# cliangyu/video-diffusion

Measured on AMD Instinct MI355X. Metric: denoise-steps/sec, higher is better.
Workload: dtype f32

## Files before the change

### video-diffusion_amd/csrc/attn_temporal.hip

```cpp
#include "vd_common.h"
#include <cstdlib>
#include <string>

namespace vd {

__device__ __forceinline__ float dot4(f32x4 a, f32x4 b) { return a.x * b.x + a.y * b.y + a.z * b.z + a.w * b.w; }

template <int PB, int TMAX, bool RPE>
__global__ __launch_bounds__(256) void attn_temporal_kernel(AttnTemporalArgs a) {
    extern __shared__ __attribute__((aligned(16))) float smem[];
    const int T = a.T, C = a.C, HW = a.HW, C3 = 3 * a.C;
    const int F = C / a.heads, F4 = F >> 2, FP = F + 4, TS = T + 1;
    float* qs = smem;
    float* ks = qs + PB * T * FP;
    float* sc = ks + PB * T * FP;
    const int b = blockIdx.z, h = blockIdx.y, p0 = blockIdx.x * PB;
    const int np = min(PB, HW - p0);
    const int tid = threadIdx.x;
    const float* qkv_b = a.qkv + (size_t)b * T * HW * C3 + h * F;

    for (int idx = tid; idx < PB * T * F4; idx += 256) {
        const int f4 = idx % F4, r = idx / F4;
        const int t = r % T, p = r / T;
        const float* src = qkv_b + ((size_t)t * HW + p0 + min(p, np - 1)) * C3 + f4 * 4;
        f32x4 q = *reinterpret_cast<const f32x4*>(src) * a.scale;
        f32x4 k = *reinterpret_cast<const f32x4*>(src + C);
        if (p >= np) { q = f32x4{0.f, 0.f, 0.f, 0.f}; k = q; }
        *reinterpret_cast<f32x4*>(qs + (p * T + t) * FP + f4 * 4) = q;
        *reinterpret_cast<f32x4*>(ks + (p * T + t) * FP + f4 * 4) = k;
    }
    __syncthreads();

    for (int pr = tid; pr < T * T; pr += 256) {
        const int t = pr / T, s = pr - t * T;
        float acc[PB];
#pragma unroll
        for (int p = 0; p < PB; ++p) acc[p] = 0.f;
        const float* rk = RPE ? a.Rk + (((size_t)b * T + t) * T + s) * C + h * F : nullptr;
        const float* rq = RPE ? a.Rq + (((size_t)b * T + s) * T + t) * C + h * F : nullptr;
        const float* qrow = qs + t * FP;
        const float* krow = ks + s * FP;
#pragma unroll 3
        for (int f0 = 0; f0 < F; f0 += 8) {
            f32x4 rk0, rk1, rq0, rq1;
            if constexpr (RPE) {
                rk0 = *reinterpret_cast<const f32x4*>(rk + f0); rk1 = *reinterpret_cast<const f32x4*>(rk + f0 + 4);
                rq0 = *reinterpret_cast<const f32x4*>(rq + f0) * a.scale; rq1 = *reinterpret_cast<const f32x4*>(rq + f0 + 4) * a.scale;
            }
#pragma unroll
            for (int p = 0; p < PB; ++p) {
                const f32x4 q0 = *reinterpret_cast<const f32x4*>(qrow + p * T * FP + f0);
                const f32x4 q1 = *reinterpret_cast<const f32x4*>(qrow + p * T * FP + f0 + 4);
                const f32x4 k0 = *reinterpret_cast<const f32x4*>(krow + p * T * FP + f0);
                const f32x4 k1 = *reinterpret_cast<const f32x4*>(krow + p * T * FP + f0 + 4);
                if constexpr (RPE)
                    acc[p] += dot4(q0, k0 + rk0) + dot4(q1, k1 + rk1) + dot4(k0, rq0) + dot4(k1, rq1);
                else
                    acc[p] += dot4(q0, k0) + dot4(q1, k1);
            }
        }
        bool masked = false;
        if (a.mask) {
            const float mt = a.mask[b * T + t], ms = a.mask[b * T + s];
            float allowed = mt * ms;
            if (a.allow_pad) allowed += (1.f - mt) * (1.f - ms);
            else if (t == s) allowed = 1.f;
            masked = allowed == 0.f;
        }
#pragma unroll
        for (int p = 0; p < PB; ++p) sc[(p * T + t) * TS + s] = masked ? -INFINITY : acc[p];
    }
    __syncthreads();

    for (int row = tid; row < np * T; row += 256) {
        float* r = sc + row * TS;
        float mx = -INFINITY;
        for (int s = 0; s < T; ++s) mx = fmaxf(mx, r[s]);
        float sum = 0.f;
        for (int s = 0; s < T; ++s) { const float e = __expf(r[s] - mx); r[s] = e; sum += e; }
        const float inv = 1.0f / sum;
        for (int s = 0; s < T; ++s) r[s] *= inv;
    }
    __syncthreads();

    for (int item = tid; item < T * F4; item += 256) {
        const int t = item / F4, f4 = item - t * F4;
        f32x4 rv[TMAX];
#pragma unroll
        for (int s = 0; s < TMAX; ++s) {
            rv[s] = f32x4{0.f, 0.f, 0.f, 0.f};
            if constexpr (RPE)
                rv[s] = *reinterpret_cast<const f32x4*>(a.Rv + (((size_t)b * T + t) * T + min(s, T - 1)) * C + h * F + f4 * 4);
        }
        for (int p = 0; p < np; ++p) {
            const float* ar = sc + (p * T + t) * TS;
            const float* vbase = qkv_b + 2 * C + (size_t)(p0 + p) * C3 + f4 * 4;
            f32x4 o = {0.f, 0.f, 0.f, 0.f};
#pragma unroll
            for (int s = 0; s < TMAX; ++s) {
                const f32x4 v = *reinterpret_cast<const f32x4*>(vbase + (size_t)min(s, T - 1) * HW * C3);
                const float w = s < T ? ar[min(s, T - 1)] : 0.f;
                o += (v + rv[s]) * w;
            }
            *reinterpret_cast<f32x4*>(a.out + (((size_t)b * T + t) * HW + p0 + p) * C + h * F + f4 * 4) = o;
        }
    }
}

#ifdef VD_ATT_TIMING
__device__ unsigned long long g_att_stamp[16];
#define ATT_STAMP(i)                                                                                   \
    do {                                                                                               \
        if (threadIdx.x == 0 && blockIdx.x == 3 && blockIdx.y == 1 && blockIdx.z == 2) {               \
            __builtin_amdgcn_sched_barrier(0);                                                         \
            g_att_stamp[i] = __builtin_amdgcn_s_memrealtime();                                         \
            __builtin_amdgcn_sched_barrier(0);                                                         \
        }                                                                                              \
    } while (0)
extern "C" int vd_debug_att_stamps(unsigned long long* host_out) {
    return (int)hipMemcpyFromSymbol(host_out, HIP_SYMBOL(g_att_stamp), sizeof(g_att_stamp));
}
#else
#define ATT_STAMP(i)
#endif

__device__ __forceinline__ f32x4 mfma4(float x, float y, f32x4 c) { return __builtin_amdgcn_mfma_f32_16x16x4f32(x, y, c, 0, 0, 0); }

__device__ __forceinline__ void rows_regs_transpose(float& x0, float& x1, float& x2, float& x3) {
    auto u = [](float f) { return __builtin_bit_cast(unsigned, f); };
    auto f = [](unsigned v) { return __builtin_bit_cast(float, v); };
    auto p01 = __builtin_amdgcn_permlane16_swap(u(x0), u(x1), false, false);
    auto p23 = __builtin_amdgcn_permlane16_swap(u(x2), u(x3), false, false);
    auto q02 = __builtin_amdgcn_permlane32_swap(p01[0], p23[0], false, false);
    auto q13 = __builtin_amdgcn_permlane32_swap(p01[1], p23[1], false, false);
    x0 = f(q02[0]); x2 = f(q02[1]); x1 = f(q13[0]); x3 = f(q13[1]);
}

template <int NT, int JM, bool RPE, bool EXACT>
__global__ __launch_bounds__(512, 2) void attn_temporal_mfma_kernel(AttnTemporalArgs a) {
    constexpr int TP = 16 * NT, RS = TP + 1, PS = TP * RS + (NT == 1 ? 1 : 17);
    extern __shared__ __attribute__((aligned(16))) float smem[];
    float* w = smem;
    const int T = EXACT ? 16 * NT : a.T, C = a.C, HW = a.HW, C3 = 3 * a.C;
    const int F = C / a.heads, NJ = EXACT ? JM : F >> 4;
    const int b = blockIdx.z, h = blockIdx.y, p0 = blockIdx.x * 16;
    const int tid = threadIdx.x, wv = tid >> 6, l = tid & 63, i16 = l & 15, g = l >> 4;
    const float* qb = a.qkv + ((size_t)b * T * HW + p0) * C3 + h * F;
    auto row = [&](int t, int px) { return qb + ((size_t)t * HW + px) * C3; };
    auto ld4 = [](const float* p) { return *reinterpret_cast<const f32x4*>(p); };
    const int tcl[2] = {min(i16, T - 1), min(16 + i16, T - 1)};
    const f32x4 zero4 = {0.f, 0.f, 0.f, 0.f};

    ATT_STAMP(0);
    constexpr int JG = NT == 1 ? 2 : 1, NG = JM / JG, NU = 2 * NT;
    constexpr bool AHEAD = NT == 1;
    struct Ops { f32x4 qa1[2][NT][JG], kb1[2][NT][JG], xa2[NU][JG], rb2[NU][NT][JG], xa3[NU][JG], rb3[NU][NT][JG]; };
    f32x4 acc1[2][NT][NT], acc2[NU][NT], acc3[NU][NT];
#pragma unroll
    for (int u = 0; u < 2; ++u)
#pragma unroll
        for (int m = 0; m < NT; ++m)
#pragma unroll
            for (int n = 0; n < NT; ++n) acc1[u][m][n] = zero4;
#pragma unroll
    for (int u = 0; u < NU; ++u)
#pragma unroll
        for (int n = 0; n < NT; ++n) { acc2[u][n] = zero4; acc3[u][n] = zero4; }
    const float* q1[2][NT];
#pragma unroll
    for (int u = 0; u < 2; ++u)
#pragma unroll
        for (int m = 0; m < NT; ++m) q1[u][m] = row(tcl[m], 2 * wv + u) + 4 * g;
    const float* rkq[NT];
#pragma unroll
    for (int n = 0; n < NT; ++n) rkq[n] = (size_t)b * T * T * C + (size_t)tcl[n] * C + h * F + 4 * g + (const float*)nullptr;
    auto request = [&](Ops& o, int grp, bool own, bool rel) {
#pragma unroll
        for (int jj = 0; jj < JG; ++jj) {
            const int j = grp * JG + jj;
            if (EXACT || j < NJ) {
                if (own) {
#pragma unroll
                    for (int u = 0; u < 2; ++u)
#pragma unroll
                        for (int m = 0; m < NT; ++m) { o.qa1[u][m][jj] = ld4(q1[u][m] + 16 * j); o.kb1[u][m][jj] = ld4(q1[u][m] + C + 16 * j); }
                }
                if constexpr (RPE) {
#pragma unroll
                    for (int u = 0; u < (rel ? NU : 0); ++u) {
                        const int t = wv + 8 * u;
                        if (EXACT || t < T) {
                            const float* xr = row(t, i16) + 4 * g + 16 * j;
                            o.xa2[u][jj] = ld4(xr);
                            o.xa3[u][jj] = ld4(xr + C);
#pragma unroll
                            for (int n = 0; n < NT; ++n) {
                                const size_t ro = (size_t)(rkq[n] - (const float*)nullptr) + (size_t)t * T * C + 16 * j;
                                o.rb2[u][n][jj] = ld4(a.Rk + ro);
                                o.rb3[u][n][jj] = ld4(a.Rq + ro);
                            }
                        }
                    }
                }
            }
        }
    };
    auto products = [&](const Ops& o, int grp, bool own, bool rel) {
#pragma unroll
        for (int jj = 0; jj < JG; ++jj) {
            if (EXACT || grp * JG + jj < NJ) {
#pragma unroll
                for (int e = 0; e < 4; ++e) {
#pragma unroll
                    for (int u = 0; u < (own ? 2 : 0); ++u)
#pragma unroll
                        for (int m = 0; m < NT; ++m)
#pragma unroll
                            for (int n = 0; n < NT; ++n) acc1[u][m][n] = mfma4(o.qa1[u][m][jj][e] * a.scale, o.kb1[u][n][jj][e], acc1[u][m][n]);
                    if constexpr (RPE) {
#pragma unroll
                        for (int u = 0; u < (rel ? NU : 0); ++u)
                            if (EXACT || wv + 8 * u < T) {
#pragma unroll
                                for (int n = 0; n < NT; ++n) {
                                    acc2[u][n] = mfma4(o.xa2[u][jj][e] * a.scale, o.rb2[u][n][jj][e], acc2[u][n]);
                                    acc3[u][n] = mfma4(o.xa3[u][jj][e], o.rb3[u][n][jj][e] * a.scale, acc3[u][n]);
                                }
                            }
                    }
                }
            }
        }
    };
    if constexpr (AHEAD) {
        Ops o[2];
        request(o[0], 0, true, true);
#pragma unroll
        for (int grp = 0; grp < NG; ++grp) {
            if (grp + 1 < NG) request(o[(grp + 1) & 1], grp + 1, true, true);
            __builtin_amdgcn_sched_barrier(0);
            products(o[grp & 1], grp, true, true);
            __builtin_amdgcn_sched_barrier(0);
        }
    } else {
#pragma unroll 1
        for (int grp = 0; grp < NG; ++grp) {
            Ops o;
            request(o, grp, true, false);
            products(o, grp, true, false);
            if constexpr (RPE) {
                request(o, grp, false, true);
                products(o, grp, false, true);
            }
        }
    }
    ATT_STAMP(1);
#pragma unroll
    for (int u = 0; u < 2; ++u)
#pragma unroll
        for (int m = 0; m < NT; ++m)
#pragma unroll
            for (int n = 0; n < NT; ++n)
#pragma unroll
                for (int r = 0; r < 4; ++r) w[(2 * wv + u) * PS + (16 * m + 4 * g + r) * RS + 16 * n + i16] = acc1[u][m][n][r];
    __syncthreads();
    if constexpr (RPE) {
#pragma unroll
        for (int u = 0; u < NU; ++u) {
            const int t = wv + 8 * u;
            if (t < T) {
#pragma unroll
                for (int n = 0; n < NT; ++n)
#pragma unroll
                    for (int r = 0; r < 4; ++r) w[(4 * g + r) * PS + t * RS + 16 * n + i16] += acc2[u][n][r];
            }
        }
        __syncthreads();
#pragma unroll
        for (int u = 0; u < NU; ++u) {
            const int sk = wv + 8 * u;
            if (sk < T) {
#pragma unroll
                for (int n = 0; n < NT; ++n)
#pragma unroll
                    for (int r = 0; r < 4; ++r) w[(4 * g + r) * PS + (16 * n + i16) * RS + sk] += acc3[u][n][r];
            }
        }
        __syncthreads();
    }

    ATT_STAMP(2);
    for (int rix = tid; rix < 16 * TP; rix += 512) {
        const int px = rix / TP, t = rix - px * TP;
        float* r = w + px * PS + t * RS;
        if (t >= T) {
            for (int s = 0; s < TP; ++s) r[s] = 0.f;
            continue;
        }
        float mx = -INFINITY;
        const float mt = a.mask ? a.mask[b * T + t] : 1.f;
        for (int s = 0; s < T; ++s) {
            float v = r[s];
            if (a.mask) {
                const float ms = a.mask[b * T + s];
                float allowed = mt * ms;
                if (a.allow_pad) allowed += (1.f - mt) * (1.f - ms);
                else if (t == s) allowed = 1.f;
                if (allowed == 0.f) v = -INFINITY;
            }
            r[s] = v;
            mx = fmaxf(mx, v);
        }
        float sum = 0.f;
        for (int s = 0; s < T; ++s) { const float e = __expf(r[s] - mx); r[s] = e; sum += e; }
        const float inv = 1.0f / sum;
        for (int s = 0; s < T; ++s) r[s] *= inv;
        for (int s = T; s < TP; ++s) r[s] = 0.f;
    }
    __syncthreads();

    ATT_STAMP(3);
    const int KS = (T + 3) >> 2;
    if (EXACT ? wv < JM : wv < NJ) {
        const int f0 = 16 * wv + i16;
        const float* vb = qb + 2 * C + f0;
        const float* rvb = RPE ? a.Rv + ((size_t)b * T) * T * C + h * F + f0 : nullptr;
#pragma unroll 1
        for (int m = 0; m < NT; ++m) {
            if (16 * m >= T) break;
            float rr[NT == 1 ? 4 : 1][16];
            f32x4 acc[16];
#pragma unroll
            for (int px = 0; px < 16; ++px) acc[px] = zero4;
#pragma unroll 1
            for (int kc = 0; kc < NT; ++kc) {
                if (16 * kc >= T) break;
                float vr[4][16];
#pragma unroll
                for (int k4 = 0; k4 < 4; ++k4)
                    if (EXACT || 4 * kc + k4 < KS) {
                        const float* vs = vb + (size_t)min(16 * kc + 4 * k4 + g, T - 1) * HW * C3;
#pragma unroll
                        for (int px = 0; px < 16; ++px) vr[k4][px] = vs[(size_t)px * C3];
                    }
                if constexpr (RPE && NT == 1) {
#pragma unroll
                    for (int k4 = 0; k4 < 4; ++k4)
                        if (EXACT || k4 < KS) {
                            const float* rv = rvb + (size_t)min(4 * k4 + g, T - 1) * C;
#pragma unroll
                            for (int tl = 0; tl < 16; ++tl) rr[k4][tl] = rv[(size_t)min(tl, T - 1) * T * C];
                        }
                }
                __builtin_amdgcn_sched_barrier(0);
#pragma unroll
                for (int k4 = 0; k4 < 4; ++k4)
                    if (EXACT || 4 * kc + k4 < KS) {
                        const float* ar = w + (16 * m + i16) * RS + 16 * kc + 4 * k4 + g;
#pragma unroll
                        for (int px = 0; px < 16; ++px) acc[px] = mfma4(ar[px * PS], vr[k4][px], acc[px]);
                    }
            }
            ATT_STAMP(4);
            f32x4 res[16];
#pragma unroll
            for (int bq = 0; bq < 4; ++bq)
#pragma unroll
                for (int d = 0; d < 4; ++d) {
                    float x0 = acc[bq][d], x1 = acc[4 + bq][d], x2 = acc[8 + bq][d], x3 = acc[12 + bq][d];
                    rows_regs_transpose(x0, x1, x2, x3);
                    res[d][bq] = x0; res[4 + d][bq] = x1; res[8 + d][bq] = x2; res[12 + d][bq] = x3;
                }
            if constexpr (RPE) {
                if constexpr (NT == 1) {
#pragma unroll
                    for (int k4 = 0; k4 < 4; ++k4)
                        if (EXACT || k4 < KS) {
                            const float* ar = w + i16 * PS + 4 * k4 + g;
#pragma unroll
                            for (int tl = 0; tl < 16; ++tl) res[tl] = mfma4(ar[tl * RS], rr[k4][tl], res[tl]);
                        }
                } else {
#pragma unroll 1
                    for (int kc = 0; kc < NT; ++kc) {
                        if (16 * kc >= T) break;
                        float r4[4][16];
#pragma unroll
                        for (int k4 = 0; k4 < 4; ++k4)
                            if (4 * kc + k4 < KS) {
                                const float* rv = rvb + (size_t)min(16 * kc + 4 * k4 + g, T - 1) * C;
#pragma unroll
                                for (int tl = 0; tl < 16; ++tl) r4[k4][tl] = rv[(size_t)min(16 * m + tl, T - 1) * T * C];
                            }
#pragma unroll
                        for (int k4 = 0; k4 < 4; ++k4)
                            if (4 * kc + k4 < KS) {
                                const float* ar = w + i16 * PS + (16 * m) * RS + 16 * kc + 4 * k4 + g;
#pragma unroll
                                for (int tl = 0; tl < 16; ++tl) res[tl] = mfma4(ar[tl * RS], r4[k4][tl], res[tl]);
                            }
                    }
                }
            }
            ATT_STAMP(5);
#pragma unroll
            for (int tl = 0; tl < 16; ++tl) {
                const int t = 16 * m + tl;
                if (t < T) {
                    float* o = a.out + (((size_t)b * T + t) * HW + p0 + 4 * g) * C + h * F + f0;
#pragma unroll
                    for (int r = 0; r < 4; ++r) o[(size_t)r * C] = res[tl][r];
                }
            }
        }
    }
    ATT_STAMP(6);
}

template <int NT, int JM, bool RPE, bool EXACT>
static int launch_tm(const AttnTemporalArgs& a, hipStream_t s) {
    constexpr int TP = 16 * NT, PS = TP * (TP + 1) + (NT == 1 ? 1 : 17);
    constexpr size_t lds = (size_t)16 * PS * sizeof(float);
    if (lds > 48 * 1024) VD_RAISE_LDS((&attn_temporal_mfma_kernel<NT, JM, RPE, EXACT>), lds);
    dim3 grid(a.HW / 16, a.heads, a.B);
    hipLaunchKernelGGL((attn_temporal_mfma_kernel<NT, JM, RPE, EXACT>), grid, dim3(512), lds, s, a);
    VD_HIP(hipGetLastError());
    return 0;
}

template <int PB, int TMAX, bool RPE>
static int launch_tt(const AttnTemporalArgs& a, size_t lds, hipStream_t s) {
    VD_RAISE_LDS((&attn_temporal_kernel<PB, TMAX, RPE>), lds);
    dim3 grid((a.HW + PB - 1) / PB, a.heads, a.B);
    hipLaunchKernelGGL((attn_temporal_kernel<PB, TMAX, RPE>), grid, dim3(256), lds, s, a);
    VD_HIP(hipGetLastError());
    return 0;
}

int launch_attn_temporal(const AttnTemporalArgs& a, hipStream_t s) {
    VD_REQUIRE(a.T >= 1 && a.T <= kMaxWindowFrames, "temporal window of 1..128 frames");
    VD_REQUIRE(a.C % a.heads == 0 && (a.C / a.heads) % 8 == 0, "head dim multiple of 8");
    VD_REQUIRE((a.Rk == nullptr) == (a.Rq == nullptr) && (a.Rk == nullptr) == (a.Rv == nullptr), "all or no RPE terms");
    if (a.T > 32) return launch_attn_temporal_long(a, s);
    const int F = a.C / a.heads;
    if (a.HW % 16 == 0 && F % 16 == 0 && F <= 128) {
        const bool rpe = a.Rk != nullptr;
        if (a.T == 16 && F == 96) return rpe ? launch_tm<1, 6, true, true>(a, s) : launch_tm<1, 6, false, true>(a, s);
        if (a.T == 16 && F == 128) return rpe ? launch_tm<1, 8, true, true>(a, s) : launch_tm<1, 8, false, true>(a, s);
        if (a.T <= 16) {
            if (F <= 64) return rpe ? launch_tm<1, 4, true, false>(a, s) : launch_tm<1, 4, false, false>(a, s);
            return rpe ? launch_tm<1, 8, true, false>(a, s) : launch_tm<1, 8, false, false>(a, s);
        }
        if (F <= 64) return rpe ? launch_tm<2, 4, true, false>(a, s) : launch_tm<2, 4, false, false>(a, s);
        return rpe ? launch_tm<2, 8, true, false>(a, s) : launch_tm<2, 8, false, false>(a, s);
    }
    auto lds_for = [&](int pb) { return ((size_t)2 * pb * a.T * (F + 4) + (size_t)pb * a.T * (a.T + 1)) * sizeof(float); };
    const bool rpe = a.Rk != nullptr;
    const bool big = lds_for(4) > 96 * 1024;
    VD_REQUIRE(lds_for(2) <= 150 * 1024, "head dim too large for the temporal attention tile");
    if (a.T <= 16) {
        if (big) return rpe ? launch_tt<2, 16, true>(a, lds_for(2), s) : launch_tt<2, 16, false>(a, lds_for(2), s);
        return rpe ? launch_tt<4, 16, true>(a, lds_for(4), s) : launch_tt<4, 16, false>(a, lds_for(4), s);
    }
    if (big) return rpe ? launch_tt<2, 32, true>(a, lds_for(2), s) : launch_tt<2, 32, false>(a, lds_for(2), s);
    return rpe ? launch_tt<4, 32, true>(a, lds_for(4), s) : launch_tt<4, 32, false>(a, lds_for(4), s);
}

}
```

Before: 49.81.

## Add low-register DUO path for exact T=16 RPE temporal attention

For the exact T=16, RPE, single-tile configuration, the kernel now targets 4 blocks per CU instead of 2. To fit that register budget it uses 32-bit byte offsets for addressing, halves the per-group operand staging, and reuses one buffer for the Rk/Rq operands. The AV and RPE-V phase is rewritten as a 16-stage software pipeline that prefetches one stage ahead and does the transpose in the middle. Dispatch now falls back to the generic path when tensor sizes exceed 32-bit offsets. Risks are register spilling and reduced load-ahead depth hurting latency hiding.

```diff
diff --git a/video-diffusion_amd/csrc/attn_temporal.hip b/video-diffusion_amd/csrc/attn_temporal.hip
--- a/video-diffusion_amd/csrc/attn_temporal.hip
+++ b/video-diffusion_amd/csrc/attn_temporal.hip
@@ -1,6 +1,7 @@
 #include "vd_common.h"
 #include <cstdlib>
 #include <string>
+#include <type_traits>
 
 namespace vd {
 
@@ -107,6 +108,9 @@
     }
 }
 
+#ifndef VD_ATT_DUO
+#define VD_ATT_DUO 1
+#endif
 #ifdef VD_ATT_TIMING
 __device__ unsigned long long g_att_stamp[16];
 #define ATT_STAMP(i)                                                                                   \
@@ -137,22 +141,25 @@
 }
 
 template <int NT, int JM, bool RPE, bool EXACT>
-__global__ __launch_bounds__(512, 2) void attn_temporal_mfma_kernel(AttnTemporalArgs a) {
+__global__ __launch_bounds__(512, (NT == 1 && RPE && EXACT && VD_ATT_DUO) ? 4 : 2) void attn_temporal_mfma_kernel(AttnTemporalArgs a) {
+    constexpr bool DUO = NT == 1 && RPE && EXACT && VD_ATT_DUO;
     constexpr int TP = 16 * NT, RS = TP + 1, PS = TP * RS + (NT == 1 ? 1 : 17);
     extern __shared__ __attribute__((aligned(16))) float smem[];
     float* w = smem;
     const int T = EXACT ? 16 * NT : a.T, C = a.C, HW = a.HW, C3 = 3 * a.C;
     const int F = C / a.heads, NJ = EXACT ? JM : F >> 4;
     const int b = blockIdx.z, h = blockIdx.y, p0 = blockIdx.x * 16;
-    const int tid = threadIdx.x, wv = tid >> 6, l = tid & 63, i16 = l & 15, g = l >> 4;
+    const int tid = threadIdx.x, wv = __builtin_amdgcn_readfirstlane(tid >> 6), l = tid & 63, i16 = l & 15, g = l >> 4;
     const float* qb = a.qkv + ((size_t)b * T * HW + p0) * C3 + h * F;
-    auto row = [&](int t, int px) { return qb + ((size_t)t * HW + px) * C3; };
+    using Off = std::conditional_t<DUO, unsigned, size_t>;
+    auto ld4o = [](const float* p, Off o) { return *reinterpret_cast<const f32x4*>(reinterpret_cast<const char*>(p) + o); };
+    auto ld1o = [](const float* p, Off o) { return *reinterpret_cast<const float*>(reinterpret_cast<const char*>(p) + o); };
     auto ld4 = [](const float* p) { return *reinterpret_cast<const f32x4*>(p); };
     const int tcl[2] = {min(i16, T - 1), min(16 + i16, T - 1)};
     const f32x4 zero4 = {0.f, 0.f, 0.f, 0.f};
 
     ATT_STAMP(0);
-    constexpr int JG = NT == 1 ? 2 : 1, NG = JM / JG, NU = 2 * NT;
+    constexpr int JG = NT == 1 && !DUO ? 2 : 1, NG = JM / JG, NU = 2 * NT;
     constexpr bool AHEAD = NT == 1;
     struct Ops { f32x4 qa1[2][NT][JG], kb1[2][NT][JG], xa2[NU][JG], rb2[NU][NT][JG], xa3[NU][JG], rb3[NU][NT][JG]; };
     f32x4 acc1[2][NT][NT], acc2[NU][NT], acc3[NU][NT];
@@ -166,38 +173,38 @@
     for (int u = 0; u < NU; ++u)
 #pragma unroll
         for (int n = 0; n < NT; ++n) { acc2[u][n] = zero4; acc3[u][n] = zero4; }
-    const float* q1[2][NT];
-#pragma unroll
-    for (int u = 0; u < 2; ++u)
-#pragma unroll
-        for (int m = 0; m < NT; ++m) q1[u][m] = row(tcl[m], 2 * wv + u) + 4 * g;
-    const float* rkq[NT];
-#pragma unroll
-    for (int n = 0; n < NT; ++n) rkq[n] = (size_t)b * T * T * C + (size_t)tcl[n] * C + h * F + 4 * g + (const float*)nullptr;
-    auto request = [&](Ops& o, int grp, bool own, bool rel) {
+    Off lo1[NT], lor[NT];
+#pragma unroll
+    for (int m = 0; m < NT; ++m) { lo1[m] = ((Off)tcl[m] * HW * C3 + 4 * g) * 4; lor[m] = ((Off)tcl[m] * C + 4 * g) * 4; }
+    const Off lox = ((Off)i16 * C3 + 4 * g) * 4;
+    auto request = [&](Ops& o, int grp, bool own, bool relx, bool relr) {
 #pragma unroll
         for (int jj = 0; jj < JG; ++jj) {
             const int j = grp * JG + jj;
             if (EXACT || j < NJ) {
                 if (own) {
 #pragma unroll
-                    for (int u = 0; u < 2; ++u)
-#pragma unroll
-                        for (int m = 0; m < NT; ++m) { o.qa1[u][m][jj] = ld4(q1[u][m] + 16 * j); o.kb1[u][m][jj] = ld4(q1[u][m] + C + 16 * j); }
+                    for (int u = 0; u < 2; ++u) {
+                        const float* q1 = qb + (size_t)(2 * wv + u) * C3 + 16 * j;
+#pragma unroll
+                        for (int m = 0; m < NT; ++m) { o.qa1[u][m][jj] = ld4o(q1, lo1[m]); o.kb1[u][m][jj] = ld4o(q1 + C, lo1[m]); }
+                    }
                 }
                 if constexpr (RPE) {
 #pragma unroll
-                    for (int u = 0; u < (rel ? NU : 0); ++u) {
+                    for (int u = 0; u < (relx || relr ? NU : 0); ++u) {
                         const int t = wv + 8 * u;
                         if (EXACT || t < T) {
-                            const float* xr = row(t, i16) + 4 * g + 16 * j;
-                            o.xa2[u][jj] = ld4(xr);
-                            o.xa3[u][jj] = ld4(xr + C);
-#pragma unroll
-                            for (int n = 0; n < NT; ++n) {
-                                const size_t ro = (size_t)(rkq[n] - (const float*)nullptr) + (size_t)t * T * C + 16 * j;
-                                o.rb2[u][n][jj] = ld4(a.Rk + ro);
-                                o.rb3[u][n][jj] = ld4(a.Rq + ro);
+                            if (relx) {
+                                const float* xr = qb + (size_t)t * HW * C3 + 16 * j;
+                                o.xa2[u][jj] = ld4o(xr, lox);
+                                o.xa3[u][jj] = ld4o(xr + C, lox);
+                            }
+                            const size_t ro = ((size_t)b * T + t) * T * C + h * F + 16 * j;
+#pragma unroll
+                            for (int n = 0; n < (relr ? NT : 0); ++n) {
+                                o.rb2[u][n][jj] = ld4o(a.Rk + ro, lor[n]);
+                                o.rb3[u][n][jj] = ld4o(a.Rq + ro, lor[n]);
                             }
                         }
                     }
@@ -205,7 +212,7 @@
             }
         }
     };
-    auto products = [&](const Ops& o, int grp, bool own, bool rel) {
+    auto products = [&](const Ops& o, const Ops& r, int grp, bool own, bool rel) {
 #pragma unroll
         for (int jj = 0; jj < JG; ++jj) {
             if (EXACT || grp * JG + jj < NJ) {
@@ -223,8 +230,8 @@
                             if (EXACT || wv + 8 * u < T) {
 #pragma unroll
                                 for (int n = 0; n < NT; ++n) {
-                                    acc2[u][n] = mfma4(o.xa2[u][jj][e] * a.scale, o.rb2[u][n][jj][e], acc2[u][n]);
-                                    acc3[u][n] = mfma4(o.xa3[u][jj][e], o.rb3[u][n][jj][e] * a.scale, acc3[u][n]);
+                                    acc2[u][n] = mfma4(o.xa2[u][jj][e] * a.scale, r.rb2[u][n][jj][e], acc2[u][n]);
+                                    acc3[u][n] = mfma4(o.xa3[u][jj][e], r.rb3[u][n][jj][e] * a.scale, acc3[u][n]);
                                 }
                             }
                     }
@@ -232,25 +239,36 @@
             }
         }
     };
-    if constexpr (AHEAD) {
+    if constexpr (DUO) {
         Ops o[2];
-        request(o[0], 0, true, true);
+        request(o[0], 0, true, true, true);
 #pragma unroll
         for (int grp = 0; grp < NG; ++grp) {
-            if (grp + 1 < NG) request(o[(grp + 1) & 1], grp + 1, true, true);
+            if (grp + 1 < NG) request(o[(grp + 1) & 1], grp + 1, true, true, false);
             __builtin_amdgcn_sched_barrier(0);
-            products(o[grp & 1], grp, true, true);
+            products(o[grp & 1], o[0], grp, true, true);
+            __builtin_amdgcn_sched_barrier(0);
+            if (grp + 1 < NG) request(o[0], grp + 1, false, false, true);
+        }
+    } else if constexpr (AHEAD) {
+        Ops o[2];
+        request(o[0], 0, true, true, true);
+#pragma unroll
+        for (int grp = 0; grp < NG; ++grp) {
+            if (grp + 1 < NG) request(o[(grp + 1) & 1], grp + 1, true, true, true);
+            __builtin_amdgcn_sched_barrier(0);
+            products(o[grp & 1], o[grp & 1], grp, true, true);
             __builtin_amdgcn_sched_barrier(0);
         }
     } else {
 #pragma unroll 1
         for (int grp = 0; grp < NG; ++grp) {
             Ops o;
-            request(o, grp, true, false);
-            products(o, grp, true, false);
+            request(o, grp, true, false, false);
+            products(o, o, grp, true, false);
             if constexpr (RPE) {
-                request(o, grp, false, true);
-                products(o, grp, false, true);
+                request(o, grp, false, true, true);
+                products(o, o, grp, false, true);
             }
         }
     }
@@ -323,15 +341,60 @@
     const int KS = (T + 3) >> 2;
     if (EXACT ? wv < JM : wv < NJ) {
         const int f0 = 16 * wv + i16;
-        const float* vb = qb + 2 * C + f0;
-        const float* rvb = RPE ? a.Rv + ((size_t)b * T) * T * C + h * F + f0 : nullptr;
+        const float* vb = qb + 2 * C + 16 * wv + (DUO ? 0 : i16);
+        const float* rvb = RPE ? a.Rv + ((size_t)b * T) * T * C + h * F + 16 * wv + (DUO ? 0 : i16) : nullptr;
 #pragma unroll 1
         for (int m = 0; m < NT; ++m) {
             if (16 * m >= T) break;
-            float rr[NT == 1 ? 4 : 1][16];
-            f32x4 acc[16];
+            float rr[NT == 1 && !DUO ? 4 : 1][16];
+            f32x4 acc[16], res[16];
 #pragma unroll
             for (int px = 0; px < 16; ++px) acc[px] = zero4;
+            auto transpose = [&]() {
+#pragma unroll
+                for (int bq = 0; bq < 4; ++bq)
+#pragma unroll
+                    for (int d = 0; d < 4; ++d) {
+                        float x0 = acc[bq][d], x1 = acc[4 + bq][d], x2 = acc[8 + bq][d], x3 = acc[12 + bq][d];
+                        rows_regs_transpose(x0, x1, x2, x3);
+                        res[d][bq] = x0; res[4 + d][bq] = x1; res[8 + d][bq] = x2; res[12 + d][bq] = x3;
+                    }
+            };
+            if constexpr (DUO) {
+                constexpr int AH = 1;
+                float ring[AH + 1][8];
+                auto request_b = [&](float (&o)[8], int st) {
+                    const int k4 = (st >> 1) & 3, i0 = 8 * (st & 1);
+                    if (st < 8) {
+                        const Off vs = ((Off)(4 * k4 + g) * HW * C3 + i16) * 4;
+#pragma unroll
+                        for (int i = 0; i < 8; ++i) o[i] = ld1o(vb, vs + (Off)(i0 + i) * C3 * 4);
+                    } else {
+                        const Off rv = ((Off)(4 * k4 + g) * C + i16) * 4;
+#pragma unroll
+                        for (int i = 0; i < 8; ++i) o[i] = ld1o(rvb, rv + (Off)(i0 + i) * T * C * 4);
+                    }
+                };
+#pragma unroll
+                for (int st = 0; st < AH; ++st) request_b(ring[st], st);
+#pragma unroll
+                for (int st = 0; st < 16; ++st) {
+                    if (st + AH < 16) request_b(ring[(st + AH) % (AH + 1)], st + AH);
+                    __builtin_amdgcn_sched_barrier(0);
+                    const int k4 = (st >> 1) & 3, i0 = 8 * (st & 1);
+                    if (st == 8) { ATT_STAMP(4); transpose(); }
+                    if (st < 8) {
+                        const float* ar = w + i16 * RS + 4 * k4 + g;
+#pragma unroll
+                        for (int i = 0; i < 8; ++i) acc[i0 + i] = mfma4(ar[(i0 + i) * PS], ring[st % (AH + 1)][i], acc[i0 + i]);
+                    } else {
+                        const float* ar = w + i16 * PS + 4 * k4 + g;
+#pragma unroll
+                        for (int i = 0; i < 8; ++i) res[i0 + i] = mfma4(ar[(i0 + i) * RS], ring[st % (AH + 1)][i], res[i0 + i]);
+                    }
+                    __builtin_amdgcn_sched_barrier(0);
+                }
+            } else {
 #pragma unroll 1
             for (int kc = 0; kc < NT; ++kc) {
                 if (16 * kc >= T) break;
@@ -362,15 +425,7 @@
                     }
             }
             ATT_STAMP(4);
-            f32x4 res[16];
-#pragma unroll
-            for (int bq = 0; bq < 4; ++bq)
-#pragma unroll
-                for (int d = 0; d < 4; ++d) {
-                    float x0 = acc[bq][d], x1 = acc[4 + bq][d], x2 = acc[8 + bq][d], x3 = acc[12 + bq][d];
-                    rows_regs_transpose(x0, x1, x2, x3);
-                    res[d][bq] = x0; res[4 + d][bq] = x1; res[8 + d][bq] = x2; res[12 + d][bq] = x3;
-                }
+            transpose();
             if constexpr (RPE) {
                 if constexpr (NT == 1) {
 #pragma unroll
@@ -401,6 +456,7 @@
                             }
                     }
                 }
+            }
             }
             ATT_STAMP(5);
 #pragma unroll
@@ -445,8 +501,9 @@
     const int F = a.C / a.heads;
     if (a.HW % 16 == 0 && F % 16 == 0 && F <= 128) {
         const bool rpe = a.Rk != nullptr;
-        if (a.T == 16 && F == 96) return rpe ? launch_tm<1, 6, true, true>(a, s) : launch_tm<1, 6, false, true>(a, s);
-        if (a.T == 16 && F == 128) return rpe ? launch_tm<1, 8, true, true>(a, s) : launch_tm<1, 8, false, true>(a, s);
+        const bool fits32 = (size_t)a.T * a.HW * 3 * a.C * sizeof(float) < ((size_t)1 << 32);
+        if (a.T == 16 && F == 96 && fits32) return rpe ? launch_tm<1, 6, true, true>(a, s) : launch_tm<1, 6, false, true>(a, s);
+        if (a.T == 16 && F == 128 && fits32) return rpe ? launch_tm<1, 8, true, true>(a, s) : launch_tm<1, 8, false, true>(a, s);
         if (a.T <= 16) {
             if (F <= 64) return rpe ? launch_tm<1, 4, true, false>(a, s) : launch_tm<1, 4, false, false>(a, s);
             return rpe ? launch_tm<1, 8, true, false>(a, s) : launch_tm<1, 8, false, false>(a, s);
```

Measured after the change: 49.84 (median of 6 runs). About the same (+0.1%).
